# JBLanier/stratego_env

Hardware: AMD Instinct MI355X
Metric: env steps/sec (higher is better)
Workload: dtype u8

## Files before the change

stratego_env_amd/csrc/sgx_layout.h:

```cpp
#pragma once

namespace {

constexpr int OBS_CH = SGX_PO_OBS_CHANNELS;
constexpr int LUT_STRIDE = SGX_OBS_LUT_STRIDE;
constexpr int FOBS_CH = SGX_FO_OBS_CHANNELS;
constexpr int LUT_ROW_PITCH = 33, LUT_BLK = 673 , LUT_DWORDS = 2 * LUT_BLK + 2;
#ifndef SGX_WPB
#define SGX_WPB 8
#endif
#ifndef SGX_MIN_WAVES
#define SGX_MIN_WAVES 6
#endif
constexpr int QTAB_DWORDS = 2 * OBS_CH * 4, OBS_TAB_DWORDS = LUT_DWORDS + QTAB_DWORDS;
constexpr int FOBS_TAB_DWORDS = LUT_DWORDS + 2 * FOBS_CH * 4;
constexpr int NIB_ONE = 4, CODE_NONE = 0xFF, CODETAB_REC = 192, CODETAB_BYTES = 208;
constexpr int COMBAT_BYTES = 16 * 16;
enum { COMBAT_LOSE = 0, COMBAT_TIE = 1, COMBAT_WIN = 2, COMBAT_WIN_FLAG = 3 };
__host__ __device__ inline int combat_outcome(int att, int def) {
    if (att == 3  && def == 12 ) return COMBAT_WIN;
    if (att == 1  && def == 10 ) return COMBAT_WIN;
    if (def == 11 ) return COMBAT_WIN_FLAG;
    if (def == 12) return COMBAT_LOSE;
    if (att == def) return COMBAT_TIE;
// ... 67 lines not shown
                             : (4 * GPW * LDS_GAME_EST + LDS_SHARED_EST <= 160 * 1024) ? 4
                             : (2 * GPW * LDS_GAME_EST + LDS_SHARED_EST <= 160 * 1024) ? 2 : 1;
};

template <int R, int C>
constexpr bool half_wave_ok() {
    using G0 = Geo<R, C>;
    return G0::LPG == 64 && !G0::WIDE && G0::RC <= 128 && (G0::ST_OFF + G0::TAIL_BYTES) / 16 <= 64;
}

struct DevTables {
    float lut[8][LUT_DWORDS];
    uint8_t obstacles[SGX_MAX_CELLS];
    alignas(16) uint8_t tmpl[4][TMPL_MAX_BYTES];
    alignas(16) uint8_t codetab[2][CODETAB_BYTES];
    alignas(16) uint8_t combat[COMBAT_BYTES];
};

#if defined(__HIP_DEVICE_COMPILE__)
#define SGX_KERNARG __attribute__((address_space(4)))
#else
#define SGX_KERNARG
#endif
template <class T>
__device__ __forceinline__ T table_entry(T const *tab, int i) {
#if defined(__HIP_DEVICE_COMPILE__)
    return ((const SGX_KERNARG T *)tab)[i];
#else
    return tab[i];
#endif
}

struct KParams {
    int8_t *boards;
    const DevTables *tab;
    const uint8_t *setups;
    int32_t n_setups;
    int32_t max_turns;
    int32_t usable_rows;
    int32_t piece_counts[12];
    int32_t rec_bytes;
    int32_t max_events;
    int64_t n_envs;
    uint64_t seed;
    int64_t env_id_offset;
    sgx_step_io io;
    int32_t mode;
    int64_t env_first;
    int32_t map_mode, map_arg;
    int32_t xcd_first[8], xcd_count[8];
    int32_t nt_stores;
    int32_t multi_ev;
    int32_t compact_stride;
    const int8_t *src_boards;
    const int32_t *src_index;
    int32_t *flag_list, *flag_count;
    int64_t traj_out_envs, traj_res_envs;
    int32_t *traj_act_log;
#ifdef SGX_STAMPS
    unsigned long long *stamps;
#endif
};

struct PoolParams {
    const int8_t *pool;
    int32_t n_pool, pool_flags;
    int32_t *start_index;
};

#ifdef SGX_STAMPS
#define STAMP(i)                                                                                   \
    do {                                                                                           \
        __builtin_amdgcn_sched_barrier(0);                                                         \
        unsigned long long t_;                                                                     \
        asm volatile("s_memtime %0\n\ts_waitcnt lgkmcnt(0)" : "=s"(t_)::"memory");                \
        __builtin_amdgcn_sched_barrier(0);                                                         \
        if (lane == 0 && P.stamps) P.stamps[env * 16 + (i)] = t_;                                  \
    } while (0)
#else
#define STAMP(i) do { } while (0)
#endif

typedef float f32x4 __attribute__((ext_vector_type(4)));
typedef int i32x4 __attribute__((ext_vector_type(4)));

template <class G, int NIB_CH = OBS_CH>
struct alignas(16) Lds {
    static constexpr int NIB_BYTES = ((G::RC * NIB_CH + 1) / 2 + 15) & ~15;
    int8_t b[N_LDS_BOARDS][G::S];
    alignas(16) uint8_t nib_lead[16];
    alignas(16) uint8_t nib[NIB_BYTES + 16];
    alignas(16) uint32_t mbits[G::MB_WORDS];
    alignas(16) uint8_t cnt[G::CNT_PAD];
    alignas(16) uint8_t occ[G::S];
    alignas(16) typename G::cell_t plist[G::CNT_PAD];
    alignas(16) uint8_t tail[G::TAIL_BYTES];
    alignas(16) float unc_val[G::EVL_MAX + G::SPECIAL_EXTRA];
    alignas(16) typename G::entry_t unc_entry[(G::EVL_MAX + G::SPECIAL_EXTRA + 7) & ~7];
};

__host__ __device__ inline uint64_t sm_fin(uint64_t z) {
    z ^= z >> 30; z *= 0xBF58476D1CE4E5B9ull;
    z ^= z >> 27; z *= 0x94D049BB133111EBull;
    z ^= z >> 31;
    return z;
}
// ... 142 lines not shown
```

stratego_env_amd/csrc/sgx_obs.h:

```cpp
#pragma once

namespace {

#ifndef SGX_OBS_UNROLL
#define SGX_OBS_UNROLL 4
#endif


__device__ inline float code_to_float(unsigned x) { return __builtin_amdgcn_cvt_off_f32_i4((int)x) * 4.0f; }

template <class G, int NB>
__device__ inline void set_code_one(Lds<G, NB> &L, int entry) {
    atomicOr(reinterpret_cast<unsigned int *>(L.nib) + (entry >> 3), (unsigned)NIB_ONE << ((entry & 7) * 4));
}
template <class G, int NB>
__device__ inline void swap_code(Lds<G, NB> &L, int entry, int was, int now) {
    atomicXor(reinterpret_cast<unsigned int *>(L.nib) + (entry >> 3), (unsigned)(was ^ now) << ((entry & 7) * 4));
}

template <class G, class Spec, int NB>
__device__ inline bool special_entry(const Lds<G, NB> &L, int i, int n_events, int rp0, int rp1, int qi, int &entry, int &ch, int &v, int &tab_idx) {
    const typename G::ev_t *evl = reinterpret_cast<const typename G::ev_t *>(L.tail + 2 * G::SB + 32);
    int cell;
    if (i < n_events) {
// ... 71 lines not shown
        }
        if (have) {
            int now, was;
            if ((G::BIG || multi) && i < n_events && v >= LUT_STRIDE) {
                const int t = (ch - Spec::CAP0) % 12, pc = piece_counts[t];
                const float hi = pc > 1 ? (float)pc : 8.0f, half = hi / 2.0f;
                val = raw ? (float)v : __fdiv_rn(__fsub_rn((float)v, half), half);
                now = CODE_NONE;
                was = codetab[16 * t];
            } else {
                now = codetab[ti];
                was = codetab[i < n_events ? (ti & ~15) : CODETAB_REC + 3];
                if (now == CODE_NONE) val = glut[lut_row(ch) + v];
            }
            if (now == CODE_NONE) { unc = true; now = CODE_ESC; }
            swap_code(L, entry, was, now);
        }
        const unsigned long long bal = gballot<G>(unc);
        if (unc) {
            const int pos = n_unc + __popcll(bal & ((1ull << lane) - 1ull));
            L.unc_entry[pos] = (typename G::entry_t)entry;
            L.unc_val[pos] = val;
        }
        n_unc += __popcll(bal);
    }
    wave_sync<G>();
    return n_unc;
}

template <class G, class Spec, int NB>
__device__ inline void store_compact(const Lds<G, NB> &L, uint8_t *__restrict__ dst, int n_unc, int lane) {
    constexpr int NBYTES = ((G::RC * Spec::NCH + 1) / 2 + 15) & ~15;
    for (int i = lane; i < NBYTES / 16; i += G::LPG) reinterpret_cast<int4 *>(dst)[i] = reinterpret_cast<const int4 *>(L.nib)[i];
    if (lane == 0) *reinterpret_cast<int4 *>(dst + NBYTES) = make_int4(n_unc, 0, 0, 0);
    uint2 *ent = reinterpret_cast<uint2 *>(dst + NBYTES + 16);
    for (int k = lane; k < n_unc; k += G::LPG) ent[k] = make_uint2((uint32_t)L.unc_entry[k], __float_as_uint(L.unc_val[k]));
}
template <class G, class Spec, int NB>
__device__ inline int load_compact(Lds<G, NB> &L, const uint8_t *__restrict__ src, int capacity, int lane) {
    constexpr int NBYTES = ((G::RC * Spec::NCH + 1) / 2 + 15) & ~15;
    for (int i = lane; i < NBYTES / 16; i += G::LPG) reinterpret_cast<int4 *>(L.nib)[i] = reinterpret_cast<const int4 *>(src)[i];
    int n_unc = reinterpret_cast<const int4 *>(src + NBYTES)->x;
    n_unc = n_unc < 0 ? 0 : (n_unc > capacity ? capacity : n_unc);
    const uint2 *ent = reinterpret_cast<const uint2 *>(src + NBYTES + 16);
    for (int k = lane; k < n_unc; k += G::LPG) {
        const uint2 e = ent[k];
        L.unc_entry[k] = (typename G::entry_t)e.x;
        L.unc_val[k] = __uint_as_float(e.y);
    }
    wave_sync<G>();
    return n_unc;
}

template <class G, class Spec, bool CHECKED, bool NT, int STRIDE = G::LPG, int NB>
__device__ inline void emit_codes(const Lds<G, NB> &L, float *__restrict__ dst, int lane) {
    constexpr int RC = G::RC, NCH = Spec::NCH;
    const uint16_t *n16 = reinterpret_cast<const uint16_t *>(L.nib);
    if constexpr (RC % 4 == 0) {
        constexpr int NQ = (RC / 4) * NCH;
        const int m0 = (int)((reinterpret_cast<uintptr_t>(dst) >> 4) & (G::LPG - 1));
        f32x4 *base = reinterpret_cast<f32x4 *>(dst);
        const int l0 = (int)((reinterpret_cast<uintptr_t>(dst) >> 4) & 7);
        const int first_line = l0 ? 0 : -1, last_line = ((l0 + NQ) & 7) ? (NQ - 1 + l0) >> 3 : -1;
        auto sweep = [&](const int q0) __attribute__((always_inline)) {
            const int q = q0 + lane;
#ifdef SGX_MUTANT_OBS_QUAD_OVER
            const bool in = (unsigned)q <= (unsigned)NQ;
#else
            const bool in = (unsigned)q < (unsigned)NQ;
#endif
            const unsigned x = n16[in ? q : 0];
            f32x4 o = {code_to_float(x), code_to_float(x >> 4), code_to_float(x >> 8), code_to_float(x >> 12)};
            bool esc = false;
            if constexpr (CHECKED) {
                const unsigned y = x ^ (0x1111u * CODE_ESC);
                esc = ((y - 0x1111u) & ~y & 0x8888u) != 0;
            }
            if constexpr (NT) {
                bool edge = ((q + l0) >> 3) == first_line || ((q + l0) >> 3) == last_line;
                if constexpr (CHECKED) {
                    const unsigned line_esc = (unsigned)(__ballot(in && esc) >> (__lane_id() & ~7)) & 0xFFu;
                    edge = edge || line_esc != 0;
                }
                if (in && !esc && edge) base[q] = o;
                if (in && !esc && !edge) __builtin_nontemporal_store(o, &base[q]);
            } else {
                if (in && !esc) base[q] = o;
            }
        };
        if constexpr (CHECKED && NT) {
            for (int q0 = -m0; q0 < NQ; q0 += STRIDE) sweep(q0);
        } else {
#pragma unroll SGX_OBS_UNROLL
            for (int q0 = -m0; q0 < NQ; q0 += STRIDE) sweep(q0);
        }
    } else {
        static_assert(!CHECKED, "odd boards patch single floats after a wait (patch_uncoded_floats)");
        static_assert(STRIDE == G::LPG, "odd boards are emitted by the game's own lanes");
        constexpr int NF = RC * NCH;
        const int a = (int)((reinterpret_cast<uintptr_t>(dst) >> 2) & 3);
        float *base = dst - a;
        const int nslots = (a + NF + 3) >> 2;
        const int m0 = (int)((reinterpret_cast<uintptr_t>(base) >> 4) & (G::LPG - 1));
        const int sh = a ? (4 - a) * 4 : 0, back = a ? 1 : 0;
        const int l0 = (int)((reinterpret_cast<uintptr_t>(base) >> 4) & 7), last_line = (nslots - 1 + l0) >> 3;
#pragma unroll 2
        for (int k0 = -m0; k0 < nslots; k0 += G::LPG) {
            const int k = k0 + lane;
            const bool slot_in = k >= 0 && k < nslots;
            const int kk = slot_in ? k : 0;
            const unsigned w = (unsigned)n16[kk - back] | ((unsigned)n16[kk - back + 1] << 16);
            const unsigned x = w >> sh;
            const float o[4] = {code_to_float(x), code_to_float(x >> 4), code_to_float(x >> 8), code_to_float(x >> 12)};
            const int f0 = 4 * kk - a;
#ifdef SGX_MUTANT_OBS_LAST_SLOT_WHOLE
            if (slot_in && f0 >= 0) {
#else
            if (slot_in && f0 >= 0 && f0 + 3 < NF) {
#endif
                f32x4 qv = {o[0], o[1], o[2], o[3]};
                const int line = (k + l0) >> 3;
                if (NT && line != 0 && line != last_line) __builtin_nontemporal_store(qv, &reinterpret_cast<f32x4 *>(base)[k]);
                else reinterpret_cast<f32x4 *>(base)[k] = qv;
            } else if (slot_in) {
#pragma unroll
                for (int j = 0; j < 4; ++j)
                    if ((unsigned)(f0 + j) < (unsigned)NF) base[4 * k + j] = o[j];
            }
        }
    }
}

// ... 125 lines not shown
```

stratego_env_amd/csrc/sgx_step.h:

```cpp
#pragma once

namespace {

template <class G, int KIND>
constexpr int tmpl_bytes(bool full) { return ((G::RC * (full ? FOBS_CH : OBS_CH) + 1) / 2 + 15) & ~15; }
template <class G, int KIND>
constexpr int tmpl_lds_bytes(bool full) { return G::WIDE ? 0 : tmpl_bytes<G, KIND>(full); }
template <class G, int KIND>
constexpr int shared_table_bytes() {
    constexpr bool FULL = (KIND & 1) != 0, ORIG = (KIND & 2) != 0;
    if (ObsKind<KIND>::NOOBS) return 16;
    if (ORIG) return 4 * (OBS_TAB_DWORDS + (FULL ? FOBS_TAB_DWORDS : 0));
    return tmpl_lds_bytes<G, KIND>(false) + (FULL ? tmpl_lds_bytes<G, KIND>(true) : 0) + CODETAB_BYTES;
}

template <class G, int KIND, bool MAPPED = false>
constexpr int waves_per_simd() {
    constexpr int per_wg = G::WPB * G::GPW * (int)sizeof(Lds<G, ObsKind<KIND>::NIB_CH>) + shared_table_bytes<G, KIND>() + G::OBST_BYTES + COMBAT_BYTES;
    constexpr int wgs = (160 * 1024) / per_wg;
    constexpr int w = wgs * G::WPB / 4;
    constexpr int want = (G::HALF || (MAPPED && ObsKind<KIND>::NOOBS)) ? 6 : (G::RC <= 64 ? 8 : SGX_MIN_WAVES);
    return w > want ? want : (w < 1 ? 1 : w);
}

// ... 421 lines not shown
    }

    STAMP(2);
    int qi = player == 1 ? 0 : 1;
    const bool want_bits = PLAY >= 5 || (PLAY < 3 && (PLAY != 0 || !NOOBS || SPLIT || io_mask != nullptr || (P.mode == 0 && P.io.next_actions_dev != nullptr)));
#ifdef SGX_ABLATE
    if (SGX_ABLATED(P.map_arg, 3)) return;
    int nvalid = gen_mask(L, qi, over, lane, P.map_arg);
#else
    int nvalid;
    if constexpr (NOOBS) nvalid = want_bits ? gen_mask(L, qi, over, lane) : gen_any(L, qi, over, lane);
    else nvalid = gen_mask(L, qi, over, lane);
#endif
    bool ended_now = false;
    if (applied && !noop_path) {
        const bool was_over = over;
        if (nvalid == 0) { over = true; flags = (flags & ~(F_WIN_P1 | F_WIN_M1)) | F_OVER | (mover == 1 ? F_WIN_P1 : F_WIN_M1); }
        if (turn >= max_turns && !over) { over = true; flags |= F_OVER | F_END_INVALID; }
        if (over && !was_over && nvalid != 0) { if (want_bits) mask_noop_only(L, lane); nvalid = 0; }
        ended_now = over;
    } else if (applied && noop_path) {
        ended_now = over;
        if (nvalid != 0) { if (want_bits) mask_noop_only(L, lane); nvalid = 0; }
    }
    flags = (flags & ~F_PLAYER_M1) | (player == -1 ? F_PLAYER_M1 : 0);
    STAMP(3);

    const bool done = over;
    const bool end_invalid = over && (flags & F_END_INVALID);
    float rew_p1 = 0.f, rew_m1 = 0.f;
    if (over && !end_invalid) {
        const int w = (flags & F_WIN_P1) ? 1 : (flags & F_WIN_M1) ? -1 : 0;
        rew_p1 = w == 0 ? 1e-4f : (float)w;
        rew_m1 = w == 0 ? 1e-4f : (float)-w;
    }
    if (!PLAY && P.mode == 0) {
        if (lane < 2 && P.io.reward_dev) P.io.reward_dev[2 * renv + lane] = lane ? rew_m1 : rew_p1;
        uint8_t *fp = lane == 0 ? P.io.done_dev : lane == 1 ? P.io.invalid_action_dev : lane == 2 ? P.io.ending_invalid_dev : nullptr;
        const uint8_t fv = lane == 0 ? (done ? 1 : 0) : lane == 1 ? (invalid_action ? 1 : 0) : (end_invalid ? 1 : 0);
        if (fp) fp[renv] = fv;
    }

    const bool raw = (P.io.flags & SGX_STEP_RAW_OBS) != 0;
    const float *glut_p = P.tab->lut[(ORIG ? 4 : 0) + (raw ? 2 : 0)], *glut_f = P.tab->lut[(ORIG ? 4 : 0) + (raw ? 2 : 0) + 1];
    const uint8_t *codetab = ORIG ? nullptr : shared + tmpl_lds_bytes<G, KIND>(false) + (FULL ? tmpl_lds_bytes<G, KIND>(true) : 0);
    auto render = [&](auto spec, bool full, int q, float *dst) -> int {
        using Spec = decltype(spec);
        if constexpr (Spec::CODES) {
            const uint8_t *tmpl = full ? shared + tmpl_lds_bytes<G, KIND>(false) : shared;
            if constexpr (G::WIDE) tmpl = P.tab->tmpl[(raw ? 2 : 0) + (full ? 1 : 0)];
            const int n_unc = build_codes<G, Spec>(L, tmpl, codetab, full ? glut_f : glut_p, q,
                                                   n_events, rp0, rp1, lane, P.piece_counts, raw, P.multi_ev != 0);
            if constexpr (RC % 4 == 0) {
                if (n_unc == 0) {
                    if (P.nt_stores) emit_codes<G, Spec, false, true>(L, dst, lane);
                    else emit_codes<G, Spec, false, false>(L, dst, lane);
                } else {
                    if (P.nt_stores) emit_codes<G, Spec, true, true>(L, dst, lane);
                    else emit_codes<G, Spec, true, false>(L, dst, lane);
                    patch_uncoded<G, Spec>(L, dst, n_unc, lane);
                }
                return 0;
            } else {
                if (P.nt_stores) emit_codes<G, Spec, false, true>(L, dst, lane);
                else emit_codes<G, Spec, false, false>(L, dst, lane);
                if (n_unc) {
                    asm volatile("s_waitcnt vmcnt(0)" ::: "memory");
                    patch_uncoded_floats(L, dst, n_unc, lane);
                }
                return 0;
            }
        } else {
            emit_obs_lut<G, Spec>(L, reinterpret_cast<const float *>(shared) + (full ? OBS_TAB_DWORDS : 0), q, dst, lane);
            if (n_events > 0) {
                asm volatile("s_waitcnt vmcnt(0)" ::: "memory");
                emit_obs_patches<G, Spec>(L, full ? glut_f : glut_p, q, dst, n_events, lane, raw, P.multi_ev != 0, P.piece_counts);
            }
            return 0;
        }
    };

    if constexpr (!NOOBS)
    if (P.mode == 0 && ended_now && P.io.final_obs_dev) {
        float *fo = P.io.final_obs_dev + env * (int64_t)(2 * RC * PS::NCH);
        render(PS{}, false, 0, fo);
        render(PS{}, false, 1, fo + RC * PS::NCH);
    }
    if constexpr (FULL)
        if (P.mode == 0 && ended_now && P.io.final_fobs_dev) {
            float *fo = P.io.final_fobs_dev + env * (int64_t)(2 * RC * FS::NCH);
            render(FS{}, true, 0, fo);
            render(FS{}, true, 1, fo + RC * FS::NCH);
        }

    bool wrote_reset = false;
    if (!PLAY && P.mode == 0 && ended_now && P.io.auto_reset) {
        game_no += 1;
        if constexpr (POOL) {
            const StartScalars st = load_start_record(L, P, *pp, env, game_no, lane);
            turn = st.turn; max_turns = st.max_turns; n_events = st.n_events; rp0 = st.rp0; rp1 = st.rp1;
            player = st.player; qi = player == 1 ? 0 : 1; over = false;
            flags = player == -1 ? F_PLAYER_M1 : 0;
        } else {
            sample_boards(L, P, (uint64_t)(P.env_id_offset + env), (uint64_t)game_no, lane);
            turn = 0; flags = 0; player = 1; qi = 0; over = false;
            n_events = 0; rp0 = rp1 = 0;
        }
        nvalid = want_bits ? gen_mask(L, qi, false, lane) : 1;
        wrote_reset = true;
    }
    if constexpr (POOL) {
// ... 321 lines not shown
```

stratego_env_amd/csrc/stratego_mi355x.hip:

```cpp
#include <hip/hip_runtime.h>
#include <type_traits>
#include <stdint.h>
#include <stdio.h>
#include <stdlib.h>
#include <sched.h>
#include <time.h>
#include <string.h>
#include <string>
#include <vector>

#include "stratego_mi355x.h"

#define SGX_API extern "C" __attribute__((visibility("default")))

namespace {

thread_local std::string g_last_error;

int fail(int code, const char *fmt, const char *detail = "") {
    char buf[512];
    snprintf(buf, sizeof(buf), fmt, detail);
    g_last_error = buf;
    return code;
}

#define HIP_TRY(expr)                                                                        \
    do {                                                                                     \
        hipError_t e_ = (expr);                                                              \
        if (e_ != hipSuccess) return fail(SGX_EDEVICE, #expr ": %s", hipGetErrorString(e_)); \
    } while (0)

struct DeviceGuard {
    int prev = -1;
    bool restore = false;
    hipError_t err = hipSuccess;
    explicit DeviceGuard(int dev) {
        err = hipGetDevice(&prev);
        if (err == hipSuccess && prev != dev) {
            err = hipSetDevice(dev);
            restore = err == hipSuccess;
        }
    }
    ~DeviceGuard() {
        if (restore) (void)hipSetDevice(prev);
    }
    DeviceGuard(const DeviceGuard &) = delete;
    DeviceGuard &operator=(const DeviceGuard &) = delete;
};
#define SGX_ON_DEVICE(dev)                                                                                      \
    DeviceGuard device_guard_(dev);                                                                             \
    if (device_guard_.err != hipSuccess) return fail(SGX_EDEVICE, "selecting the handle's device: %s", hipGetErrorString(device_guard_.err))

#ifndef SGX_BUILD_ID
#define SGX_BUILD_ID "unknown"
#endif
const char g_build_id[] = "SGX_BUILD_ID=" SGX_BUILD_ID;

}

#include "sgx_layout.h"
#include "sgx_obs.h"
#include "sgx_mask.h"
#include "sgx_setup.h"
#include "sgx_step.h"
#include "sgx_playout.h"
#include "sgx_replay.h"
#include "sgx_children.h"
#include "sgx_lane.h"
#include "sgx_lane_kernel.h"
#include "sgx_aux_kernels.h"
#include "sgx_choose.h"
#include "sgx_mem.h"


struct sgx_env {
    sgx_config cfg;
    int64_t n_envs;
    int device;
    uint64_t seed;
    int64_t env_id_offset;
    int8_t *boards;
    DevTables *tab;
    uint8_t *setups;
    int64_t n_setups;
    int rec_bytes;
    int sc_off;
    int max_events;
    int K;
    unsigned long long *stamps;
    int map_mode, map_arg;
    int xcd_skew;
    int xcd_explicit;
    int32_t xcd_w[8];
    int nt_mode;
    int lane_mode;
    float placement_target_us;
    hipStream_t chain_stream[SGX_MAX_CHAINS];
    hipEvent_t chain_fork, chain_join[SGX_MAX_CHAINS];
    uint32_t *sync_flag_host, *sync_flag_dev, *sync_count;
    uint32_t sync_seq;
    int no_single;
    uint8_t *san_flags;
    int32_t *redo_list;
    int general_states;
    int no_multi_step;
    int multi_step_attr;
    int multi_step_attr_pool;
    int last_kind;
    int multi_step_wave;
    int steps_barrier;
    int half_wave;
    void **ring_tab_dev, **ring_tab_host;
    int ring_tab_cap, ring_tab_n;
    hipEvent_t ring_tab_ev;
    hipStream_t ring_tab_stream;
    int8_t *pool;
    int64_t n_pool;
    int pool_flags;
    int32_t *start_index;
    int32_t *count_scratch;
    int64_t *scan_sums;
    int64_t count_scratch_cap, scan_sums_cap;
};

namespace {

#ifdef SGX_ONLY_EXTRA
#define SGX_BUILTIN_GEOMETRIES(X, A)
#else
#define SGX_BUILTIN_GEOMETRIES(X, A) X(A, 10, 10) X(A, 15, 15) X(A, 8, 8) X(A, 6, 6) X(A, 5, 5) X(A, 4, 4) X(A, 3, 4)
#endif
#ifdef SGX_EXTRA_R
#define SGX_EXTRA_GEOMETRY(X, A) X(A, SGX_EXTRA_R, SGX_EXTRA_C)
static_assert(SGX_EXTRA_R >= 3 && SGX_EXTRA_C >= 3 && SGX_EXTRA_R * SGX_EXTRA_C <= SGX_MAX_CELLS, "SGX_EXTRA_R x SGX_EXTRA_C out of range");
#else
#define SGX_EXTRA_GEOMETRY(X, A)
#endif
#define SGX_ALL_GEOMETRIES(X, A) SGX_BUILTIN_GEOMETRIES(X, A) SGX_EXTRA_GEOMETRY(X, A)

bool supported_geometry(int r, int c) {
#define SGX_MATCH(A, R, C) if (r == (R) && c == (C)) return true;
    SGX_ALL_GEOMETRIES(SGX_MATCH, _)
#undef SGX_MATCH
    return false;
}

template <int N> using int_c = std::integral_constant<int, N>;
// ... 178 lines not shown
                return fail(SGX_EINVAL, "recent-move channels are normalised differently%s");
            ct[CODETAB_REC + v] = (uint8_t)float_code(f);
        }
    }
    return SGX_OK;
}

SGX_API int sgx_build_obs_lut(const sgx_config *cfg, float *lut) {
    if (int rc = check_cfg(cfg)) return rc;
    if (!lut) return fail(SGX_EINVAL, "lut is NULL%s");
    build_lut(cfg, false, lut);
    return SGX_OK;
}

SGX_API int sgx_build_full_obs_lut(const sgx_config *cfg, float *lut) {
    if (int rc = check_cfg(cfg)) return rc;
    if (!lut) return fail(SGX_EINVAL, "lut is NULL%s");
    build_lut(cfg, true, lut);
    return SGX_OK;
}

SGX_API int sgx_build_original_obs_lut(const sgx_config *cfg, int32_t full, float *lut) {
    if (int rc = check_cfg(cfg)) return rc;
    if (!lut) return fail(SGX_EINVAL, "lut is NULL%s");
    build_lut(cfg, full != 0, lut, false, true);
    return SGX_OK;
}

SGX_API int sgx_create(const sgx_config *cfg, int64_t n_envs, int device, uint64_t seed, int64_t env_id_offset, sgx_env **out) {
    if (!out) return fail(SGX_EINVAL, "out is NULL%s");
    *out = nullptr;
    if (int rc = check_cfg(cfg)) return rc;
    if (!supported_geometry(cfg->rows, cfg->cols))
        return fail(SGX_EINVAL, "board size not compiled into this library (built in: 10x10, 15x15, 8x8, 6x6, 5x5, 4x4, 3x4; any other size: "
                                "build the same sources with -DSGX_EXTRA_R=<rows> -DSGX_EXTRA_C=<cols>, stratego_env_amd/build.py build_geometry)%s");
    if (n_envs <= 0 || n_envs > (int64_t)1 << 30) return fail(SGX_EINVAL, "n_envs out of range%s");
    int ndev = 0;
    hipError_t e = hipGetDeviceCount(&ndev);
    if (e != hipSuccess || ndev <= 0) return fail(SGX_EDEVICE, "no HIP device available: %s", hipGetErrorString(e));
    if (device < 0 || device >= ndev) return fail(SGX_EINVAL, "device index out of range%s");
    SGX_ON_DEVICE(device);
    sgx_env *h = new sgx_env();
    memset(h, 0, sizeof(*h));
    h->cfg = *cfg;
    h->n_envs = n_envs;
    h->device = device;
    h->seed = seed;
    h->env_id_offset = env_id_offset;
    h->nt_mode = -1;
    if (const char *e = getenv("SGX_NT")) {
        if (!strcmp(e, "0")) h->nt_mode = 0;
        else if (!strcmp(e, "1")) h->nt_mode = 1;
    }
    h->lane_mode = -1;
    h->general_states = 1;
    if (const char *e = getenv("SGX_GENERAL_STATES")) h->general_states = atoi(e);
    if (const char *e = getenv("SGX_LANE")) { if (!strcmp(e, "0")) h->lane_mode = 0; else if (!strcmp(e, "1")) h->lane_mode = 1; }
    h->xcd_skew = -1;
    if (const char *e = getenv("SGX_XCD_SKEW")) { if (strcmp(e, "auto")) h->xcd_skew = atoi(e); }
    if (h->xcd_skew > 900) h->xcd_skew = 900;
    if (const char *e = getenv("SGX_NO_SINGLE")) h->no_single = atoi(e);
    if (const char *e = getenv("SGX_MULTI_STEP")) h->no_multi_step = !strcmp(e, "0");
    h->multi_step_wave = 1;
    if (const char *e = getenv("SGX_MULTI_STEP_WAVE")) h->multi_step_wave = strcmp(e, "0") != 0;
    h->half_wave = 1;
    if (const char *e = getenv("SGX_HALF_WAVE")) h->half_wave = strcmp(e, "0") != 0;
    h->steps_barrier = -1;
    if (const char *e = getenv("SGX_STEPS_BARRIER")) h->steps_barrier = !strcmp(e, "0") ? 0 : !strcmp(e, "1") ? 1 : -1;
    if (const char *e = getenv("SGX_MAP")) { h->map_mode = atoi(e); if (const char *c = strchr(e, ',')) h->map_arg = atoi(c + 1); }
    const int rc_cells = cfg->rows * cfg->cols;
    {
        int pieces = 0;
        for (int i = 0; i < 12; ++i) pieces += cfg->piece_counts[i];
        if (cfg->capture_capacity > pieces) pieces = cfg->capture_capacity;
        h->max_events = 2 * pieces;
        if (h->max_events > rc_cells) h->max_events = rc_cells;
        const int st_off = (STORED_BOARDS * ((rc_cells + 3) & ~3) + 15) & ~15, sb = (((rc_cells + 7) / 8) + 15) & ~15;
        const int sc_off = st_off + 2 * sb;
        h->sc_off = sc_off;
        h->rec_bytes = (sc_off + 32 + (rc_cells > 256 ? 4 : 2) * h->max_events + 127) & ~127;
    }
    h->K = 2 * (cfg->rows - 1) + 2 * (cfg->cols - 1) + 1;
    DevTables host_tab;
    memset(&host_tab, 0, sizeof(host_tab));
    {
        float dense[FOBS_CH * LUT_STRIDE];
        for (int k = 0; k < 8; ++k) {
            const bool original = (k & 4) != 0, raw = (k & 2) != 0, full = (k & 1) != 0;
            build_lut(cfg, full, dense, raw, original);
            for (int ch = 0; ch < lut_channels(full, original); ++ch)
                for (int i = 0; i < LUT_STRIDE; ++i) host_tab.lut[k][lut_row(ch) + i] = dense[ch * LUT_STRIDE + i];
        }
    }
    memcpy(host_tab.obstacles, cfg->obstacles, rc_cells);
    if (int rc = build_code_tables(cfg, &host_tab)) { delete h; return rc; }
    for (int a = 0; a < 16; ++a)
        for (int d = 0; d < 16; ++d) host_tab.combat[16 * a + d] = (uint8_t)combat_outcome(a, d);
    if (hipMalloc((void **)&h->boards, (size_t)n_envs * h->rec_bytes) != hipSuccess ||
        hipMalloc((void **)&h->tab, sizeof(DevTables)) != hipSuccess) {
        sgx_destroy(h);
        return fail(SGX_ENOMEM, "device allocation failed%s");
    }
#define HIP_TRY_OR_DESTROY(expr)                                                             \
    do {                                                                                     \
        hipError_t e_ = (expr);                                                              \
        if (e_ != hipSuccess) { sgx_destroy(h); return fail(SGX_EDEVICE, #expr ": %s", hipGetErrorString(e_)); } \
// ... 161 lines not shown
        for (int64_t i = 0; i < n_pool; ++i) { sc[8 * i] = 0; sc[8 * i + 2] = h->cfg.max_turns; }
        e = hipMemcpy2D(buf_dev + h->sc_off, (size_t)h->rec_bytes, sc.data(), 32, 32, (size_t)n_pool, hipMemcpyHostToDevice);
    }
    if (e == hipSuccess) e = hipDeviceSynchronize();
    if (e != hipSuccess) { (void)hipFree(buf_dev); return fail(SGX_EDEVICE, "sgx_set_start_pool: %s", hipGetErrorString(e)); }
    if (h->pool) (void)hipFree(h->pool);
    h->pool = buf_dev;
    h->n_pool = n_pool;
    h->pool_flags = flags & SGX_POOL_RANDOM_FIRST_PLAYER;
    return SGX_OK;
}

SGX_API int sgx_set_start_index_out(sgx_env *h, int32_t *start_index_dev) {
    if (!h) return fail(SGX_EINVAL, "sgx_set_start_index_out: handle is NULL%s");
    if (int rc = check_aligned("sgx_set_start_index_out", "start_index_dev", start_index_dev, 4)) return rc;
    h->start_index = start_index_dev;
    return SGX_OK;
}

SGX_API int64_t sgx_start_pool_size(const sgx_env *h) { return (h && h->pool) ? h->n_pool : 0; }

SGX_API int sgx_reset(sgx_env *h, const uint8_t *env_select_dev, const int8_t *p1_maps_dev, const int8_t *p2_maps_dev, void *stream) {
    if (!h) return fail(SGX_EINVAL, "handle is NULL%s");
    if ((p1_maps_dev == nullptr) != (p2_maps_dev == nullptr)) return fail(SGX_EINVAL, "pass both piece maps or neither%s");
    if (!p1_maps_dev)
        if (int rc = check_random_setups(h)) return rc;
    SGX_ON_DEVICE(h->device);
    if (h->pool) {
        const KParams p = make_params(h);
        const PoolParams pp = make_pool_params(h);
        const unsigned grid = (unsigned)h->n_envs;
        if (!p1_maps_dev) {
            reset_pool_kernel<<<grid, 64, 0, (hipStream_t)stream>>>(p, pp, env_select_dev, h->sc_off);
            HIP_TRY(hipGetLastError());
            return SGX_OK;
        }
        if (pp.start_index) {
            start_index_none_kernel<<<(grid + 255) / 256, 256, 0, (hipStream_t)stream>>>(pp.start_index, env_select_dev, h->n_envs);
            HIP_TRY(hipGetLastError());
        }
    }
    ResetParams rp;
    rp.k = make_params(h);
    rp.select = env_select_dev;
    rp.p1_maps = p1_maps_dev;
    rp.p2_maps = p2_maps_dev;
    if (int rc = for_geometry(h, [&](auto r, auto c) {
            reset_kernel<decltype(r)::value, decltype(c)::value><<<(unsigned)h->n_envs, 64, 0, (hipStream_t)stream>>>(rp);
        })) return rc;
    HIP_TRY(hipGetLastError());
    return SGX_OK;
}

constexpr int64_t CACHE_FIT_BYTES = (int64_t)300 * 1000 * 1000;
static bool past_cache(int64_t bytes) { return bytes > CACHE_FIT_BYTES; }
static int nt_for(const sgx_env *h, int64_t bytes) { return h->nt_mode < 0 ? (past_cache(bytes) ? 1 : 0) : h->nt_mode; }

static int64_t launch_obs_bytes(const sgx_env *h, const KParams &p) {
    const bool original = (p.io.flags & SGX_STEP_ORIGINAL_CHANNELS) != 0;
    const int64_t cells = (int64_t)h->cfg.rows * h->cfg.cols;
    int64_t bytes = 0;
    if (p.io.obs_dev) bytes += h->n_envs * cells * lut_channels(false, original) * 4;
    if (p.io.fobs_dev) bytes += h->n_envs * cells * lut_channels(true, original) * 4;
    return bytes;
}

#define SGX_XCD_SKEW_DEFAULT 100
static unsigned shares_for(KParams &p, int64_t groups, const int32_t *w) {
    int64_t sum = 0, cnt[8], given = 0;
    for (int x = 0; x < 8; ++x) sum += w[x];
    for (int x = 0; x < 8; ++x) { cnt[x] = groups * w[x] / sum; given += cnt[x]; }
    for (int x = 0; given < groups; x = (x + 1) & 7) { cnt[x] += 1; given += 1; }
    int64_t at = 0, mx = 1;
    for (int x = 0; x < 8; ++x) {
        p.xcd_first[x] = (int32_t)at;
        p.xcd_count[x] = (int32_t)cnt[x];
        at += cnt[x];
        if (cnt[x] > mx) mx = cnt[x];
    }
    return (unsigned)(8 * mx);
}
static void launch_shares(const sgx_env *h, bool streaming, int32_t *w) {
    if (h->xcd_explicit) { for (int x = 0; x < 8; ++x) w[x] = h->xcd_w[x]; return; }
    const int cells = h->cfg.rows * h->cfg.cols;
    const int skew = h->xcd_skew < 0 ? ((streaming && cells >= 64 && cells <= 100) ? SGX_XCD_SKEW_DEFAULT : 0) : h->xcd_skew;
    for (int x = 0; x < 8; ++x) w[x] = (x & 1) ? 1000 - skew : 1000 + skew;
}

static void launch_setup(const sgx_env *h, KParams &p, int sets, int32_t *w) {
    p.map_mode = h->map_mode; p.map_arg = h->map_arg;
    const int64_t bytes = launch_obs_bytes(h, p) * sets;
    p.nt_stores = nt_for(h, bytes);
    launch_shares(h, past_cache(bytes), w);
}
static unsigned grid_for(KParams &p, int64_t games, const int32_t *w) { return shares_for(p, (p.n_envs - p.env_first + games - 1) / games, w); }
template <class G>
unsigned geo_grid(KParams &p, const int32_t *w) { return grid_for(p, G::WPB * G::GPW, w); }

template <int R, int C, int KIND, class F>
void with_half_wave(const sgx_env *h, F &&f) {
    if constexpr (KIND == 8 && half_wave_ok<R, C>())
        if (h->half_wave) return f(int_c<2>());
    f(int_c<0>());
}

static bool lane_eligible(const sgx_env *h, const KParams &p, bool full, bool original, bool multi_step = false) {
    const int cells = h->cfg.rows * h->cfg.cols;
    auto aligned = [](const void *ptr, uintptr_t a) { return (reinterpret_cast<uintptr_t>(ptr) & (a - 1)) == 0; };
    if (h->lane_mode < 0 && p.io.obs_dev && !multi_step) return false;
    return h->lane_mode != 0 && !p.multi_ev && !(p.io.flags & (SGX_STEP_COMPACT_OBS | SGX_STEP_COMPACT_MASK)) && cells <= 16 && cells % 4 == 0 && !full && !original && h->map_mode == 0 &&
           !(p.io.flags & (SGX_STEP_MASK_1D | SGX_STEP_MASK_STATE_COORDS)) && !p.src_boards && !p.io.final_obs_dev && !p.io.final_fobs_dev &&
           (h->rec_bytes == 128 || h->rec_bytes == 256) && (p.env_first & 63) == 0 &&
           aligned(p.io.obs_dev, 16) && aligned(p.io.mask_dev, 16) && aligned(p.io.reward_dev, 8) && aligned(p.io.actions_dev, 16);
}

static int check_step_io(sgx_env *h, const KParams &p) {
    if (p.mode == 0 && p.io.auto_reset) return check_random_setups(h);
    return SGX_OK;
}

static int check_aligned(const char *fn, const char *name, const void *ptr, int align) {
    if ((reinterpret_cast<uintptr_t>(ptr) & (uintptr_t)(align - 1)) == 0) return SGX_OK;
    char buf[160];
    snprintf(buf, sizeof(buf), "%s: %s must be %d-byte aligned", fn, name, align);
    return fail(SGX_EINVAL, "%s", buf);
}
static int check_io_pointers(const sgx_env *h, const sgx_step_io &io, const char *fn) {
    const int quad = (h->cfg.rows * h->cfg.cols) % 4 == 0 ? 16 : 4;
    const struct { const char *name; const void *ptr; int align; } tab[] = {
        {"actions_dev", io.actions_dev, (io.flags & SGX_STEP_ACTIONS_POSITIONS) ? 16 : 4},
        {"obs_dev", io.obs_dev, (io.flags & SGX_STEP_COMPACT_OBS) ? 16 : quad},
        {"fobs_dev", io.fobs_dev, quad},
        {"mask_dev", io.mask_dev, (io.flags & SGX_STEP_COMPACT_MASK) ? 16 : 1},
        {"reward_dev", io.reward_dev, 4},
        {"done_dev", io.done_dev, 1},
        {"player_dev", io.player_dev, 1},
        {"invalid_action_dev", io.invalid_action_dev, 1},
        {"ending_invalid_dev", io.ending_invalid_dev, 1},
        {"final_obs_dev", io.final_obs_dev, quad},
        {"final_fobs_dev", io.final_fobs_dev, quad},
        {"next_actions_dev", io.next_actions_dev, 4},
    };
    for (const auto &e : tab)
        if (int rc = check_aligned(fn, e.name, e.ptr, e.align)) return rc;
    return SGX_OK;
// ... 95 lines not shown
    auto misaligned = [](const sgx_step_io &io) { return ((reinterpret_cast<uintptr_t>(io.obs_dev) | reinterpret_cast<uintptr_t>(io.mask_dev)) & 15) != 0; };
    if (compact && (full || io0.final_obs_dev)) return false;
    if (compact && misaligned(io0)) return false;
    if (no_obs && h->cfg.rows * h->cfg.cols <= 12 && lane_eligible(h, p, false, false)) return false;
    if (sets.strided) return !(compact && ((sets.obs_b | sets.mask_b) & 15));
    for (int32_t k = 0; k < sets.n_sets; ++k) {
        const sgx_step_io &io = sets.ios[k];
        if (io.final_obs_dev != io0.final_obs_dev || io.final_fobs_dev != io0.final_fobs_dev || (io.obs_dev == nullptr) != (io0.obs_dev == nullptr) ||
            (io.fobs_dev == nullptr) != (io0.fobs_dev == nullptr) || (io.mask_dev == nullptr) != (io0.mask_dev == nullptr)) return false;
        if (compact && misaligned(io)) return false;
    }
    return true;
}

static bool sets_share_results(const OutSets &sets, const sgx_step_io &io0) {
    if (sets.strided) return true;
    for (int32_t k = 0; k < sets.n_sets; ++k) {
        const sgx_step_io &io = sets.ios[k];
        if (io.reward_dev != io0.reward_dev || io.done_dev != io0.done_dev || io.player_dev != io0.player_dev || io.invalid_action_dev != io0.invalid_action_dev ||
            io.ending_invalid_dev != io0.ending_invalid_dev) return false;
    }
    return true;
}

static int steps_launch(sgx_env *h, StepsParams &sp, KParams &p, const int32_t *w, hipStream_t stream, bool *ok) {
    *ok = false;
    return for_geometry(h, [&](auto r, auto c) {
        constexpr int R = decltype(r)::value, C = decltype(c)::value;
        if constexpr (lane_geometry<Geo<R, C>>()) {
            const unsigned grid = grid_for(p, 64, w);
            const size_t dyn = 2 * 64 * (size_t)(p.rec_bytes + 16);
            auto raise_lds = [&](const void *kernel, int &done) {
                if (dyn + sizeof(StepsLds<Geo<R, C>>) <= 64 * 1024 || done) return true;
                if (hipFuncSetAttribute(kernel, hipFuncAttributeMaxDynamicSharedMemorySize, (int)dyn) != hipSuccess) {
                    (void)hipGetLastError();
                    h->no_multi_step = 1;
                    return false;
                }
                done = 1;
                return true;
            };
            if (!raise_lds(reinterpret_cast<const void *>(&lane_steps_kernel<R, C>), h->multi_step_attr)) return;
            sp.k = p;
            if (h->pool) {
                if (!raise_lds(reinterpret_cast<const void *>(&lane_steps_kernel_pool<R, C>), h->multi_step_attr_pool)) return;
                lane_steps_kernel_pool<R, C><<<grid, 64 * (1 + KSTEP_EMITTERS), dyn, stream>>>(sp, make_pool_params(h));
            } else
                lane_steps_kernel<R, C><<<grid, 64 * (1 + KSTEP_EMITTERS), dyn, stream>>>(sp);
            *ok = true;
        }
    });
}

static int steps_launch(sgx_env *h, WaveStepsParams &sp, KParams &p, const int32_t *w, hipStream_t stream, bool *ok) {
    const sgx_step_io &io = p.io;
    const bool compact = (io.flags & (SGX_STEP_COMPACT_OBS | SGX_STEP_COMPACT_MASK)) != 0;
    const bool no_obs = !io.obs_dev && !io.fobs_dev && !io.final_obs_dev && !io.final_fobs_dev && !compact;
    const int kind = compact ? 4 : no_obs ? 8 : (io.fobs_dev || io.final_fobs_dev) ? 1 : 0;
    const int cells = h->cfg.rows * h->cfg.cols;
    const bool pays = (kind == 0 || kind == 1) && cells >= 36 && cells <= 225 && sp.n_sets >= (cells == 100 ? WSTEPS_MAX_SETS + 1 : 16);
    const bool want_barrier = h->steps_barrier > 0 || (h->steps_barrier < 0 && pays);
    *ok = true;
    return for_geometry(h, [&](auto r, auto c) {
        constexpr int R = decltype(r)::value, C = decltype(c)::value;
        auto launch = [&](auto kind_c) {
            constexpr int KIND = decltype(kind_c)::value;
            with_half_wave<R, C, KIND>(h, [&](auto var) {
                constexpr int VAR = decltype(var)::value;
                using G = Geo<R, C, VAR>;
                const unsigned grid = geo_grid<G>(p, w);
                sp.k = p;
                sp.barrier = want_barrier && (p.n_envs - p.env_first) % (G::WPB * G::GPW) == 0;
                if (h->pool) steps_kernel_pool<R, C, KIND, VAR><<<grid, 64 * G::WPB, 0, stream>>>(WaveStepsParamsPool{sp, make_pool_params(h)});
                else steps_kernel<R, C, KIND, VAR><<<grid, 64 * G::WPB, 0, stream>>>(sp);
            });
        };
        if (kind == 0) launch(int_c<0>());
        else if (kind == 1) launch(int_c<1>());
        else if (kind == 4) launch(int_c<4>());
        else launch(int_c<8>());
    });
}

template <class SP>
static int multi_step(sgx_env *h, const KParams &p_in, const OutSets &sets, int32_t first, int32_t n_steps, void *stream, bool *launched) {
    constexpr bool lane = std::is_same<SP, StepsParams>::value;
    *launched = false;
    const int32_t n_sets = sets.n_sets;
    KParams p = p_in;
    p.mode = 0;
    p.io = sets.ios[sets.strided ? 0 : first];
    if (n_steps < 2 || h->no_multi_step || !(lane ? lane_steps_ok(h, p, sets) : wave_steps_ok(h, p, sets)) || !sets_share_results(sets, p.io)) return SGX_OK;
    if (int rc = check_step_io(h, p)) return rc;
    SP sp;
    memset(&sp, 0, sizeof(sp));
    sp.n_sets = n_sets;
    if (sets.strided) {
        sp.strided = 1;
        sp.obs_slot_bytes = sets.obs_b; sp.mask_slot_bytes = sets.mask_b;
        sp.obs[0] = p.io.obs_dev; sp.mask[0] = p.io.mask_dev;
        if constexpr (!lane) { sp.fobs_slot_bytes = sets.fobs_b; sp.fobs[0] = p.io.fobs_dev; }
    } else if (n_sets > (int32_t)std::extent<decltype(sp.obs)>::value) {
        void **tab = nullptr;
        if (int rc = upload_ring_table(h, sets, (hipStream_t)stream, &tab)) return rc;
        sp.strided = 2;
        sp.obs_tab = reinterpret_cast<float *const *>(tab);
        sp.mask_tab = reinterpret_cast<uint8_t *const *>(tab + 2 * n_sets);
        if constexpr (!lane) sp.fobs_tab = reinterpret_cast<float *const *>(tab + n_sets);
    } else
        for (int32_t k = 0; k < n_sets; ++k) {
            sp.obs[k] = sets.ios[k].obs_dev; sp.mask[k] = sets.ios[k].mask_dev;
            if constexpr (!lane) sp.fobs[k] = sets.ios[k].fobs_dev;
        }
    int32_t w[8];
    launch_setup(h, p, n_sets, w);
    for (int32_t done = 0; done < n_steps; ) {
        const int32_t now = n_steps - done > SGX_STEPS_MAX_PER_LAUNCH ? SGX_STEPS_MAX_PER_LAUNCH : n_steps - done;
        const int32_t set = (int32_t)(((int64_t)first + done) % n_sets);
        if (now < 2) {
            if (int rc = launch_set_step(h, p_in, sets, set, stream)) return rc;
        } else {
            sp.n_steps = now; sp.first_set = set;
            bool ok = false;
            if (int rc = steps_launch(h, sp, p, w, (hipStream_t)stream, &ok)) return rc;
            if (!ok) {
                if (done == 0) return SGX_OK;
                return fail(SGX_EDEVICE, "lane_steps_kernel became unavailable in the middle of a call%s");
            }
            HIP_TRY(hipGetLastError());
        }
        done += now;
    }
    *launched = true;
    h->last_kind = lane ? SGX_LAUNCH_MULTI_STEP : SGX_LAUNCH_MULTI_STEP_WAVE;
// ... 18 lines not shown
    KParams p = p_in;
    if (int rc = check_step_io(h, p)) return rc;
    int32_t w[8];
    launch_setup(h, p, ring_sets, w);
    const hipStream_t st = (hipStream_t)stream;
    const bool full = p.io.fobs_dev || p.io.final_fobs_dev, original = (p.io.flags & SGX_STEP_ORIGINAL_CHANNELS) != 0;
    const bool compact = (p.io.flags & (SGX_STEP_COMPACT_OBS | SGX_STEP_COMPACT_MASK)) != 0;
    const bool pool = allow_pool && h->pool != nullptr && p.mode == 0;
    const PoolParams pool_params = make_pool_params(h, start_index_off);
    if (compact) {
        if (full || original || p.io.final_obs_dev || p.src_boards || (p.io.flags & (SGX_STEP_MASK_1D | SGX_STEP_MASK_STATE_COORDS)))
            return fail(SGX_EINVAL, "compact outputs come with the 67-channel partial observation and the perspective mask only (no fobs / final_obs / original channels / state-coordinate masks)%s");
        if ((reinterpret_cast<uintptr_t>(p.io.obs_dev) | reinterpret_cast<uintptr_t>(p.io.mask_dev)) & 15)
            return fail(SGX_EINVAL, "compact outputs need 16-byte aligned obs_dev / mask_dev%s");
    }
    if (lane_eligible(h, p, full, original)) {
        if (int rc = for_geometry(h, [&](auto r, auto c) {
                constexpr int R = decltype(r)::value, C = decltype(c)::value;
                if constexpr (lane_geometry<Geo<R, C>>()) {
                    const unsigned grid = grid_for(p, 64, w);
                    const size_t dyn = 64 * (size_t)(p.rec_bytes + 16);
                    if (p.mode) lane_kernel<R, C, true><<<grid, 64, dyn, st>>>(p);
                    else if (pool) lane_kernel_pool<R, C><<<grid, 64, dyn, st>>>(p, pool_params);
                    else lane_kernel<R, C, false><<<grid, 64, dyn, st>>>(p);
                }
            })) return rc;
        HIP_TRY(hipGetLastError());
        h->last_kind = SGX_LAUNCH_LANE;
        return SGX_OK;
    }
    const bool no_obs = !p.io.obs_dev && !p.io.fobs_dev && !p.io.final_obs_dev && !p.io.final_fobs_dev && !compact;
    const bool mapped = (p.io.flags & (SGX_STEP_MASK_1D | SGX_STEP_MASK_STATE_COORDS)) || p.src_boards;
    if (mapped && (full || (original && !no_obs))) return fail(SGX_EINVAL, "state-coordinate masks and sgx_expand come with the 67-channel partial observation only%s");
    const int kind = compact ? 4 : no_obs ? 8 : (full ? 1 : 0) + (original ? 2 : 0);
    if (pool && mapped && p.io.auto_reset)
        return fail(SGX_EINVAL, "a handle with a start pool does not auto-reset in launches with state-coordinate masks (SGX_STEP_MASK_1D / _STATE_COORDS)%s");
    if (int rc = for_geometry(h, [&](auto r, auto c) {
            constexpr int R = decltype(r)::value, C = decltype(c)::value;
            auto launch = [&](auto kind_c, auto mapped_c) {
                constexpr int KIND = decltype(kind_c)::value;
                constexpr bool MAPPED = decltype(mapped_c)::value;
                with_half_wave<R, C, KIND>(h, [&](auto var) {
                    constexpr int VAR = decltype(var)::value;
                    using G = Geo<R, C, VAR>;
                    const unsigned grid = geo_grid<G>(p, w);
                    if (p.mode) observe_kernel<R, C, KIND, MAPPED, VAR><<<grid, 64 * G::WPB, 0, st>>>(p);
                    else if constexpr (!MAPPED) {
                        if (pool) {
                            WaveStepsParams sp;
                            memset(&sp, 0, sizeof(sp));
                            sp.k = p;
                            sp.k.traj_res_envs = sp.k.traj_out_envs = 0;
                            sp.k.traj_act_log = nullptr;
                            sp.n_steps = sp.n_sets = 1;
                            sp.obs[0] = p.io.obs_dev; sp.fobs[0] = p.io.fobs_dev; sp.mask[0] = p.io.mask_dev;
                            steps_kernel_pool<R, C, KIND, VAR><<<grid, 64 * G::WPB, 0, st>>>(WaveStepsParamsPool{sp, pool_params});
                        } else step_kernel<R, C, KIND, MAPPED, VAR><<<grid, 64 * G::WPB, 0, st>>>(p);
                    } else step_kernel<R, C, KIND, MAPPED, VAR><<<grid, 64 * G::WPB, 0, st>>>(p);
                });
            };
            if (mapped) {
                if (kind == 8) launch(int_c<8>(), bool_c<true>());
                else launch(int_c<0>(), bool_c<true>());
            } else if (kind == 0) launch(int_c<0>(), bool_c<false>());
            else if (kind == 1) launch(int_c<1>(), bool_c<false>());
            else if (kind == 2) launch(int_c<2>(), bool_c<false>());
            else if (kind == 3) launch(int_c<3>(), bool_c<false>());
            else if (kind == 4) launch(int_c<4>(), bool_c<false>());
            else launch(int_c<8>(), bool_c<false>());
        })) return rc;
    HIP_TRY(hipGetLastError());
    h->last_kind = SGX_LAUNCH_WAVE;
    return SGX_OK;
}

SGX_API int sgx_observe(sgx_env *h, float *obs_dev, float *fobs_dev, uint8_t *mask_dev, int8_t *player_dev, int32_t flags, void *stream) {
    if (!h) return fail(SGX_EINVAL, "handle is NULL%s");
    SGX_ON_DEVICE(h->device);
    KParams p = make_params(h);
    p.mode = 1;
    p.io.obs_dev = obs_dev;
    p.io.fobs_dev = fobs_dev;
    p.io.flags = flags & (SGX_STEP_RAW_OBS | SGX_STEP_ORIGINAL_CHANNELS | SGX_STEP_MASK_1D | SGX_STEP_MASK_STATE_COORDS | SGX_STEP_COMPACT_OBS | SGX_STEP_COMPACT_MASK);
    p.io.mask_dev = mask_dev;
    p.io.player_dev = player_dev;
    if (int rc = check_io_pointers(h, p.io, "sgx_observe")) return rc;
    return launch_step(h, p, stream);
}

namespace {
struct EventPair {
    hipEvent_t e0 = nullptr, e1 = nullptr;
    hipError_t err;
    EventPair() {
        err = hipEventCreate(&e0);
        if (err == hipSuccess) err = hipEventCreate(&e1);
    }
    ~EventPair() {
        if (e0) (void)hipEventDestroy(e0);
        if (e1) (void)hipEventDestroy(e1);
    }
    EventPair(const EventPair &) = delete;
    EventPair &operator=(const EventPair &) = delete;
    template <class F>
    int time(hipStream_t stream, int32_t launches, const char *what, float *ms, F &&launch) {
        if (int rc = launch()) return rc;
// ... 977 lines not shown
```

Before: 263.2 million.

## Add cache-budget store policy splitting observation lines between plain and nontemporal stores

Adds a host-side store policy for multi-step launches. It estimates the rewrite set of resident games against a cache budget and either turns nontemporal stores off entirely or marks a prefix of observation cache lines for plain stores. The observation emitter gains a compile-time SPLIT mode that sends lines below plain_lines through normal stores, so part of the output can stay cache-resident while the rest bypasses the cache. The policy adds occupancy queries on first use, and its budget heuristics may misjudge the actual cache behaviour.

Result: faster. 275.6 million (median of 6 runs) (+4.7%).

```diff
diff --git a/stratego_env_amd/csrc/sgx_layout.h b/stratego_env_amd/csrc/sgx_layout.h
--- a/stratego_env_amd/csrc/sgx_layout.h
+++ b/stratego_env_amd/csrc/sgx_layout.h
@@ -143,6 +143,7 @@
     int32_t nt_stores;
     int32_t multi_ev;
     int32_t compact_stride;
+    int16_t plain_lines;
     const int8_t *src_boards;
     const int32_t *src_index;
     int32_t *flag_list, *flag_count;
diff --git a/stratego_env_amd/csrc/sgx_obs.h b/stratego_env_amd/csrc/sgx_obs.h
--- a/stratego_env_amd/csrc/sgx_obs.h
+++ b/stratego_env_amd/csrc/sgx_obs.h
@@ -147,8 +147,8 @@
     return n_unc;
 }
 
-template <class G, class Spec, bool CHECKED, bool NT, int STRIDE = G::LPG, int NB>
-__device__ inline void emit_codes(const Lds<G, NB> &L, float *__restrict__ dst, int lane) {
+template <class G, class Spec, bool CHECKED, bool NT, int STRIDE = G::LPG, bool SPLIT = false, int NB>
+__device__ inline void emit_codes(const Lds<G, NB> &L, float *__restrict__ dst, int lane, int plain_lines = 0) {
     constexpr int RC = G::RC, NCH = Spec::NCH;
     const uint16_t *n16 = reinterpret_cast<const uint16_t *>(L.nib);
     if constexpr (RC % 4 == 0) {
@@ -173,6 +173,7 @@
             }
             if constexpr (NT) {
                 bool edge = ((q + l0) >> 3) == first_line || ((q + l0) >> 3) == last_line;
+                if constexpr (SPLIT) edge = edge || ((q + l0) >> 3) < plain_lines;
                 if constexpr (CHECKED) {
                     const unsigned line_esc = (unsigned)(__ballot(in && esc) >> (__lane_id() & ~7)) & 0xFFu;
                     edge = edge || line_esc != 0;
diff --git a/stratego_env_amd/csrc/sgx_step.h b/stratego_env_amd/csrc/sgx_step.h
--- a/stratego_env_amd/csrc/sgx_step.h
+++ b/stratego_env_amd/csrc/sgx_step.h
@@ -497,11 +497,14 @@
             const int n_unc = build_codes<G, Spec>(L, tmpl, codetab, full ? glut_f : glut_p, q,
                                                    n_events, rp0, rp1, lane, P.piece_counts, raw, P.multi_ev != 0);
             if constexpr (RC % 4 == 0) {
+                constexpr bool SPLIT_LINES = PERSIST_ != 0 && PLAY == 0 && KIND == 0;
+                int plain_lines = 0;
+                if constexpr (SPLIT_LINES) plain_lines = P.plain_lines;
                 if (n_unc == 0) {
-                    if (P.nt_stores) emit_codes<G, Spec, false, true>(L, dst, lane);
+                    if (P.nt_stores) emit_codes<G, Spec, false, true, G::LPG, SPLIT_LINES>(L, dst, lane, plain_lines);
                     else emit_codes<G, Spec, false, false>(L, dst, lane);
                 } else {
-                    if (P.nt_stores) emit_codes<G, Spec, true, true>(L, dst, lane);
+                    if (P.nt_stores) emit_codes<G, Spec, true, true, G::LPG, SPLIT_LINES>(L, dst, lane, plain_lines);
                     else emit_codes<G, Spec, true, false>(L, dst, lane);
                     patch_uncoded<G, Spec>(L, dst, n_unc, lane);
                 }
diff --git a/stratego_env_amd/csrc/sgx_store_policy.h b/stratego_env_amd/csrc/sgx_store_policy.h
--- /dev/null
+++ b/stratego_env_amd/csrc/sgx_store_policy.h
@@ -0,0 +1,64 @@
+#ifndef SGX_STORE_POLICY_H
+#define SGX_STORE_POLICY_H
+#include <stdint.h>
+
+#define SGX_CACHE_FIT_BYTES ((int64_t)300 * 1000 * 1000)
+#define SGX_PLAIN_BUDGET_BYTES ((int64_t)250 * 1000 * 1000)
+#define SGX_STORE_SPLIT_DEFAULT 1
+#define SGX_STORE_LINE_BYTES 128
+#define SGX_STORE_SWEEP_LINES 8
+#define SGX_RESULT_BYTES 12
+
+typedef struct sgx_store_shape {
+    int32_t cus;
+    int32_t wg_per_cu;
+    int32_t games_per_wg;
+    int64_t games;
+    int32_t sets;
+    int64_t obs_bytes, fobs_bytes, mask_bytes;
+    int64_t budget;
+    int32_t split;
+} sgx_store_shape;
+
+typedef struct sgx_store_policy {
+    int32_t nt_stores;
+    int32_t plain_lines;
+    int32_t fobs_plain_lines;
+} sgx_store_policy;
+
+static inline int32_t sgx_store_lines(int64_t bytes) { return (int32_t)((bytes + SGX_STORE_LINE_BYTES - 1) / SGX_STORE_LINE_BYTES); }
+static inline int32_t sgx_store_max_plain_lines(int64_t bytes) { return sgx_store_lines(bytes) / SGX_STORE_SWEEP_LINES * SGX_STORE_SWEEP_LINES; }
+
+static inline int sgx_store_fits_launch(int64_t launch_bytes_times_sets) { return launch_bytes_times_sets <= SGX_CACHE_FIT_BYTES; }
+
+static inline int64_t sgx_store_resident_games(const sgx_store_shape *s) {
+    const int64_t resident = (int64_t)s->cus * s->wg_per_cu * s->games_per_wg;
+    return resident < s->games ? resident : s->games;
+}
+static inline int64_t sgx_store_rewrite_set(const sgx_store_shape *s) {
+    return sgx_store_resident_games(s) * s->sets * (s->obs_bytes + s->fobs_bytes + s->mask_bytes + SGX_RESULT_BYTES);
+}
+
+static inline sgx_store_policy sgx_store_policy_multi_step(const sgx_store_shape *s) {
+    sgx_store_policy out = {1, 0, 0};
+    if (sgx_store_rewrite_set(s) <= s->budget) {
+        out.nt_stores = 0;
+        out.plain_lines = sgx_store_max_plain_lines(s->obs_bytes);
+        out.fobs_plain_lines = sgx_store_max_plain_lines(s->fobs_bytes);
+        return out;
+    }
+    if (!s->split) return out;
+    const int64_t slots = sgx_store_resident_games(s) * s->sets;
+    const int64_t per = slots > 0 ? s->budget / slots - s->mask_bytes - SGX_RESULT_BYTES : 0;
+    const int64_t sweep = (int64_t)SGX_STORE_SWEEP_LINES * SGX_STORE_LINE_BYTES;
+    int64_t sweeps = per > 0 ? per / sweep : 0;
+    const int64_t obs_sweeps = sgx_store_max_plain_lines(s->obs_bytes) / SGX_STORE_SWEEP_LINES;
+    const int64_t fobs_sweeps = sgx_store_max_plain_lines(s->fobs_bytes) / SGX_STORE_SWEEP_LINES;
+    const int64_t to_obs = sweeps < obs_sweeps ? sweeps : obs_sweeps;
+    sweeps -= to_obs;
+    const int64_t to_fobs = sweeps < fobs_sweeps ? sweeps : fobs_sweeps;
+    out.plain_lines = (int32_t)to_obs * SGX_STORE_SWEEP_LINES;
+    out.fobs_plain_lines = (int32_t)to_fobs * SGX_STORE_SWEEP_LINES;
+    return out;
+}
+#endif
diff --git a/stratego_env_amd/csrc/stratego_mi355x.hip b/stratego_env_amd/csrc/stratego_mi355x.hip
--- a/stratego_env_amd/csrc/stratego_mi355x.hip
+++ b/stratego_env_amd/csrc/stratego_mi355x.hip
@@ -58,6 +58,7 @@
 
 }
 
+#include "sgx_store_policy.h"
 #include "sgx_layout.h"
 #include "sgx_obs.h"
 #include "sgx_mask.h"
@@ -93,6 +94,11 @@
     int xcd_explicit;
     int32_t xcd_w[8];
     int nt_mode;
+    int plain_lines_forced;
+    int cus;
+    int steps_wg_per_cu[2][2];
+    int policy_debug;
+    int policy_printed[4];
     int lane_mode;
     float placement_target_us;
     hipStream_t chain_stream[SGX_MAX_CHAINS];
@@ -377,6 +383,16 @@
         if (!strcmp(e, "0")) h->nt_mode = 0;
         else if (!strcmp(e, "1")) h->nt_mode = 1;
     }
+    h->plain_lines_forced = -1;
+    if (const char *e = getenv("SGX_NT_PLAIN_LINES")) {
+        char *end = nullptr;
+        const long v = strtol(e, &end, 10);
+        if (end != e && *end == 0) h->plain_lines_forced = v < 0 ? -1 : v > 0x7FFF ? 0x7FFF : (int)v;
+    }
+    if (const char *e = getenv("SGX_STORE_POLICY_DEBUG")) {
+        h->policy_debug = !strcmp(e, "1");
+        h->policy_printed[0] = -1;
+    }
     h->lane_mode = -1;
     h->general_states = 1;
     if (const char *e = getenv("SGX_GENERAL_STATES")) h->general_states = atoi(e);
@@ -644,9 +660,8 @@
     return SGX_OK;
 }
 
-constexpr int64_t CACHE_FIT_BYTES = (int64_t)300 * 1000 * 1000;
-static bool past_cache(int64_t bytes) { return bytes > CACHE_FIT_BYTES; }
-static int nt_for(const sgx_env *h, int64_t bytes) { return h->nt_mode < 0 ? (past_cache(bytes) ? 1 : 0) : h->nt_mode; }
+static bool past_cache(int64_t bytes) { return !sgx_store_fits_launch(bytes); }
+static int nt_for(const sgx_env *h, int64_t bytes) { return h->nt_mode >= 0 ? h->nt_mode : h->plain_lines_forced >= 0 ? 1 : (past_cache(bytes) ? 1 : 0); }
 
 static int64_t launch_obs_bytes(const sgx_env *h, const KParams &p) {
     const bool original = (p.io.flags & SGX_STEP_ORIGINAL_CHANNELS) != 0;
@@ -683,6 +698,7 @@
     p.map_mode = h->map_mode; p.map_arg = h->map_arg;
     const int64_t bytes = launch_obs_bytes(h, p) * sets;
     p.nt_stores = nt_for(h, bytes);
+    p.plain_lines = (int16_t)((h->nt_mode < 0 && h->plain_lines_forced >= 0) ? h->plain_lines_forced : 0);
     launch_shares(h, past_cache(bytes), w);
 }
 static unsigned grid_for(KParams &p, int64_t games, const int32_t *w) { return shares_for(p, (p.n_envs - p.env_first + games - 1) / games, w); }
@@ -884,6 +900,42 @@
     });
 }
 
+template <int R, int C, int KIND>
+static int steps_policy(sgx_env *h, KParams &p, int32_t n_sets) {
+    if (h->nt_mode >= 0 || h->plain_lines_forced >= 0 || !p.nt_stores || (p.io.flags & SGX_STEP_ORIGINAL_CHANNELS)) return SGX_OK;
+    using G = Geo<R, C, 0>;
+    const int pool = h->pool ? 1 : 0;
+    if (!h->cus) {
+        int cus = 0;
+        HIP_TRY(hipDeviceGetAttribute(&cus, hipDeviceAttributeMultiprocessorCount, h->device));
+        h->cus = cus;
+    }
+    if (!h->steps_wg_per_cu[KIND][pool]) {
+        int wgs = 0;
+        if (pool) HIP_TRY(hipOccupancyMaxActiveBlocksPerMultiprocessor(&wgs, steps_kernel_pool<R, C, KIND, 0>, 64 * G::WPB, 0));
+        else HIP_TRY(hipOccupancyMaxActiveBlocksPerMultiprocessor(&wgs, steps_kernel<R, C, KIND, 0>, 64 * G::WPB, 0));
+        h->steps_wg_per_cu[KIND][pool] = wgs > 0 ? wgs : 1;
+    }
+    const int64_t cells = (int64_t)R * C;
+    sgx_store_shape s;
+    s.cus = h->cus; s.wg_per_cu = h->steps_wg_per_cu[KIND][pool]; s.games_per_wg = G::WPB * G::GPW;
+    s.games = p.n_envs - p.env_first; s.sets = n_sets;
+    s.obs_bytes = p.io.obs_dev ? cells * lut_channels(false, false) * 4 : 0;
+    s.fobs_bytes = p.io.fobs_dev ? cells * lut_channels(true, false) * 4 : 0;
+    s.mask_bytes = p.io.mask_dev ? cells * h->K : 0;
+    s.budget = SGX_PLAIN_BUDGET_BYTES; s.split = KIND == 0 ? SGX_STORE_SPLIT_DEFAULT : 0;
+    const sgx_store_policy pol = sgx_store_policy_multi_step(&s);
+    p.nt_stores = pol.nt_stores; p.plain_lines = (int16_t)(KIND == 0 ? pol.plain_lines : 0);
+    const int now[4] = {n_sets, p.nt_stores, p.plain_lines, s.wg_per_cu};
+    if (h->policy_debug && memcmp(now, h->policy_printed, sizeof(now)) != 0) {
+        memcpy(h->policy_printed, now, sizeof(now));
+        fprintf(stderr, "sgx store policy: kind %d games %lld sets %d cus %d resident_wgs_per_cu %d games_per_wg %d rewrite_set %lld budget %lld -> nt_stores %d plain_lines %d\n",
+                KIND, (long long)s.games, (int)n_sets, s.cus, s.wg_per_cu, s.games_per_wg, (long long)sgx_store_rewrite_set(&s), (long long)s.budget,
+                (int)p.nt_stores, (int)p.plain_lines);
+    }
+    return SGX_OK;
+}
+
 static int steps_launch(sgx_env *h, WaveStepsParams &sp, KParams &p, const int32_t *w, hipStream_t stream, bool *ok) {
     const sgx_step_io &io = p.io;
     const bool compact = (io.flags & (SGX_STEP_COMPACT_OBS | SGX_STEP_COMPACT_MASK)) != 0;
@@ -893,7 +945,8 @@
     const bool pays = (kind == 0 || kind == 1) && cells >= 36 && cells <= 225 && sp.n_sets >= (cells == 100 ? WSTEPS_MAX_SETS + 1 : 16);
     const bool want_barrier = h->steps_barrier > 0 || (h->steps_barrier < 0 && pays);
     *ok = true;
-    return for_geometry(h, [&](auto r, auto c) {
+    int policy_rc = SGX_OK;
+    const int geo_rc = for_geometry(h, [&](auto r, auto c) {
         constexpr int R = decltype(r)::value, C = decltype(c)::value;
         auto launch = [&](auto kind_c) {
             constexpr int KIND = decltype(kind_c)::value;
@@ -901,6 +954,9 @@
                 constexpr int VAR = decltype(var)::value;
                 using G = Geo<R, C, VAR>;
                 const unsigned grid = geo_grid<G>(p, w);
+                if constexpr ((KIND == 0 || KIND == 1) && VAR == 0 && (R * C) % 4 == 0) {
+                    if (int rc = steps_policy<R, C, KIND>(h, p, sp.n_sets)) { policy_rc = rc; return; }
+                }
                 sp.k = p;
                 sp.barrier = want_barrier && (p.n_envs - p.env_first) % (G::WPB * G::GPW) == 0;
                 if (h->pool) steps_kernel_pool<R, C, KIND, VAR><<<grid, 64 * G::WPB, 0, stream>>>(WaveStepsParamsPool{sp, make_pool_params(h)});
@@ -912,6 +968,7 @@
         else if (kind == 4) launch(int_c<4>());
         else launch(int_c<8>());
     });
+    return geo_rc ? geo_rc : policy_rc;
 }
 
 template <class SP>
@@ -1036,6 +1093,7 @@
                             sp.k = p;
                             sp.k.traj_res_envs = sp.k.traj_out_envs = 0;
                             sp.k.traj_act_log = nullptr;
+                            sp.k.plain_lines = 0;
                             sp.n_steps = sp.n_sets = 1;
                             sp.obs[0] = p.io.obs_dev; sp.fobs[0] = p.io.fobs_dev; sp.mask[0] = p.io.mask_dev;
                             steps_kernel_pool<R, C, KIND, VAR><<<grid, 64 * G::WPB, 0, st>>>(WaveStepsParamsPool{sp, pool_params});
```
